# prs-eth/Marigold

Hardware: NVIDIA B200
Metric: denoise-steps/sec @768px (UNet forward + scheduler step per ensemble member) (higher is better)
Workload: dtype bf16

## Files before the change

### marigold_b200/csrc/attn_tc.cu

```cuda
#include <cstdlib>
#include "common.cuh"
#include "kernels.h"
#include "launch.h"

namespace mgb {

constexpr int attn_threads(int rt) { return 64 + 128 * rt; }
constexpr int kQBytes = 128 * 128;
constexpr int kKvBytes = 64 * 128;
constexpr int kPBytes = 128 * 128;
constexpr int kKvStages = 3;
constexpr float kRescaleThreshold = 8.0f;
constexpr int kAttnDefaultRT = 2;
struct AttnParams {
  CUtensorMap tmap_q;
  CUtensorMap tmap_kv;
  bf16* out;
  int T, C;
  float scale_log2;
  int splits;
  float* part_o;
  float* part_ml;
};

template <int N>
__device__ __forceinline__ void quarter_barrier(int q) {
  switch (q) {
    case 0: asm volatile("bar.sync 1, %0;" ::"n"(N) : "memory"); break;
    case 1: asm volatile("bar.sync 2, %0;" ::"n"(N) : "memory"); break;
    case 2: asm volatile("bar.sync 3, %0;" ::"n"(N) : "memory"); break;
    default: asm volatile("bar.sync 4, %0;" ::"n"(N) : "memory"); break;
  }
}

template <int RT>
__global__ void __launch_bounds__(attn_threads(RT), 2) flash_attn64_kernel(const __grid_constant__ AttnParams p) {
  pdl_launch_dependents();
  extern __shared__ uint8_t smem_raw[];
  uint8_t* smem = reinterpret_cast<uint8_t*>((reinterpret_cast<uintptr_t>(smem_raw) + 1023) & ~uintptr_t(1023));
  uint8_t* sQ = smem;
  uint8_t* sK = sQ + kQBytes;
  uint8_t* sV = sK + kKvStages * kKvBytes;
  uint64_t* bars = reinterpret_cast<uint64_t*>(sV + kKvStages * kKvBytes);
  uint64_t* q_full = bars;
  uint64_t* k_full = bars + 1;
  uint64_t* k_empty = bars + 4;
  uint64_t* v_full = bars + 7;
  uint64_t* v_empty = bars + 10;
  uint64_t* s_full = bars + 13;
  uint64_t* p_full = bars + 15;
  uint64_t* p_empty = bars + 17;
  uint32_t* tmem_ptr_smem = reinterpret_cast<uint32_t*>(bars + 19);
  float* s_xch = reinterpret_cast<float*>(bars + 20);

  const int warp = threadIdx.x >> 5, lane = threadIdx.x & 31;
  const int q0 = blockIdx.x * 128, head = blockIdx.y, img = blockIdx.z / p.splits, split = blockIdx.z % p.splits;
  const int nkv_all = (p.T + 63) / 64;
  const int jb0 = split * nkv_all / p.splits;
  const int nkv = (split + 1) * nkv_all / p.splits - jb0;

  if (warp == 0 && lane == 0) {
    tma_prefetch_desc(&p.tmap_q);
    tma_prefetch_desc(&p.tmap_kv);
    mbar_init(q_full, 1);
    for (int s = 0; s < kKvStages; ++s) {
      mbar_init(&k_full[s], 1); mbar_init(&k_empty[s], 1);
      mbar_init(&v_full[s], 1); mbar_init(&v_empty[s], 1);
    }
    for (int b = 0; b < 2; ++b) {
      mbar_init(&s_full[b], 1);
      mbar_init(&p_full[b], 128 * RT);
      mbar_init(&p_empty[b], 1);
    }
    fence_mbar_init();
  }
  if (warp == 1) {
    tmem_alloc(tmem_ptr_smem, 256);
    tmem_relinquish();
  }
  tc_fence_before();
  __syncthreads();
  tc_fence_after();
  const uint32_t tmem_base = *tmem_ptr_smem;
  const uint32_t tmem_o = tmem_base + 128;
  pdl_wait();

  if (warp == 0) {
    if (elect_one()) {
      const uint32_t kfull = smem_u32(k_full), kempty = smem_u32(k_empty), vfull = smem_u32(v_full),
                     vempty = smem_u32(v_empty);
      const uint32_t sK_a = smem_u32(sK), sV_a = smem_u32(sV);
      mbar_arrive_expect_tx(q_full, kQBytes);
      tma_load_3d(sQ, &p.tmap_q, q_full, head * 64, q0, img);
      const int ck = p.C + head * 64, cv = 2 * p.C + head * 64;
      uint32_t s = 0, ph = 0;
      for (int j = 0; j < nkv; ++j) {
        mbar_wait_a(kempty + s * 8, ph ^ 1);
        mbar_expect_tx_a(kfull + s * 8, kKvBytes);
        tma_load_3d_a(sK_a + s * kKvBytes, &p.tmap_kv, kfull + s * 8, ck, (jb0 + j) * 64, img);
        mbar_wait_a(vempty + s * 8, ph ^ 1);
        mbar_expect_tx_a(vfull + s * 8, kKvBytes);
        tma_load_3d_a(sV_a + s * kKvBytes, &p.tmap_kv, vfull + s * 8, cv, (jb0 + j) * 64, img);
        if (++s == kKvStages) { s = 0; ph ^= 1; }
      }
    }
  } else if (warp == 1) {
    if (elect_one()) {
      constexpr uint32_t idesc_s = umma_idesc_bf16(128, 64, false);
      constexpr uint32_t idesc_pv = umma_idesc_bf16(128, 64, true);
      constexpr uint32_t kHi = uint32_t(kDescSw128Hi >> 32), kLbo = 1u << 16;
      const uint32_t kfull = smem_u32(k_full), kempty = smem_u32(k_empty), vfull = smem_u32(v_full),
                     vempty = smem_u32(v_empty), sfull = smem_u32(s_full), pfull = smem_u32(p_full),
                     pempty = smem_u32(p_empty);
      const uint32_t dq_lo = (smem_u32(sQ) >> 4) | kLbo, dk_lo0 = (smem_u32(sK) >> 4) | kLbo,
                     dv_lo0 = (smem_u32(sV) >> 4) | kLbo;
      uint32_t ks = 0, kph = 0, vs = 0, vph = 0;
      auto issue_s = [&](int j) {
        mbar_wait_a(kfull + ks * 8, kph);
        const uint32_t dk_lo = dk_lo0 + ks * uint32_t(kKvBytes >> 4);
        const uint32_t ts = tmem_base + uint32_t(j & 1) * 64;
        umma_bf16(ts, make_u64(dq_lo, kHi), make_u64(dk_lo, kHi), idesc_s, 0u);
        umma_bf16(ts, make_u64(dq_lo + 2, kHi), make_u64(dk_lo + 2, kHi), idesc_s, 1u);
        umma_bf16(ts, make_u64(dq_lo + 4, kHi), make_u64(dk_lo + 4, kHi), idesc_s, 1u);
        umma_bf16(ts, make_u64(dq_lo + 6, kHi), make_u64(dk_lo + 6, kHi), idesc_s, 1u);
        umma_commit_a(kempty + ks * 8);
        umma_commit_a(sfull + uint32_t(j & 1) * 8);
        if (++ks == kKvStages) { ks = 0; kph ^= 1; }
      };
      mbar_wait_a(smem_u32(q_full), 0);
      issue_s(0);
      for (int j = 0; j < nkv; ++j) {
        if (j + 1 < nkv) issue_s(j + 1);
        const uint32_t b = uint32_t(j & 1);
        mbar_wait_a(pfull + b * 8, uint32_t(j >> 1) & 1u);
        mbar_wait_a(vfull + vs * 8, vph);
        tc_fence_after();
        const uint32_t tp = tmem_base + 192 + b * 32;
        const uint32_t dv_lo = dv_lo0 + vs * uint32_t(kKvBytes >> 4);
        umma_bf16_ts(tmem_o, tp, make_u64(dv_lo, kHi), idesc_pv, j > 0 ? 1u : 0u);
        umma_bf16_ts(tmem_o, tp + 8, make_u64(dv_lo + 128, kHi), idesc_pv, 1u);
        umma_bf16_ts(tmem_o, tp + 16, make_u64(dv_lo + 256, kHi), idesc_pv, 1u);
        umma_bf16_ts(tmem_o, tp + 24, make_u64(dv_lo + 384, kHi), idesc_pv, 1u);
        umma_commit_a(vempty + vs * 8);
        umma_commit_a(pempty + b * 8);
        if (++vs == kKvStages) { vs = 0; vph ^= 1; }
      }
    }
    __syncwarp();
  } else {
    constexpr int NS = 64 / RT;
    const int q = warp & 3;
    const int h = (warp - 2) >> 2;
    const int row = q * 32 + lane;
    const uint32_t lane_off = uint32_t(q * 32) << 16;
    float m_ref = 0.f, l_run = 0.f;
    for (int j = 0; j < nkv; ++j) {
      const int b = j & 1, u = j >> 1;
      mbar_wait(&s_full[b], u & 1);
      tc_fence_after();
      uint32_t r[NS];
      TmemIO<NS>::ld(tmem_base + lane_off + b * 64 + h * NS, r);
      tmem_wait_ld();
      const int kv_valid = p.T - (jb0 + j) * 64 - h * NS;
      if (kv_valid < NS) {
#pragma unroll
        for (int i = 0; i < NS; ++i)
          if (i >= kv_valid) r[i] = 0xff800000u;
      }
      float mxa = __uint_as_float(r[0]), mxb = __uint_as_float(r[1]), mxc = __uint_as_float(r[2]),
            mxd = __uint_as_float(r[3]);
#pragma unroll
      for (int i = 4; i < NS; i += 4) {
        mxa = fmaxf(mxa, __uint_as_float(r[i]));
        mxb = fmaxf(mxb, __uint_as_float(r[i + 1]));
        mxc = fmaxf(mxc, __uint_as_float(r[i + 2]));
        mxd = fmaxf(mxd, __uint_as_float(r[i + 3]));
      }
      float mx = fmaxf(fmaxf(mxa, mxb), fmaxf(mxc, mxd));
      float* xs = s_xch + ((b * 4 + q) * RT) * 32;
      xs[h * 32 + lane] = mx;
      quarter_barrier<32 * RT>(q);
#pragma unroll
      for (int k = 1; k < RT; ++k) mx = fmaxf(mx, xs[((h + k) % RT) * 32 + lane]);
      const float m_blk = mx * p.scale_log2;
      if (j == 0) {
        m_ref = m_blk;
      } else {
        const bool need = m_blk > m_ref + kRescaleThreshold;
        if (__any_sync(0xffffffffu, need)) {
          const float m_new = need ? m_blk : m_ref;
          const float alpha = ex2_approx(m_ref - m_new);
          m_ref = m_new;
          l_run *= alpha;
          mbar_wait(&p_empty[(j - 1) & 1], ((j - 1) >> 1) & 1);
          tc_fence_after();
          uint32_t o[NS];
          TmemIO<NS>::ld(tmem_o + lane_off + h * NS, o);
          tmem_wait_ld();
#pragma unroll
          for (int i = 0; i < NS; ++i) o[i] = __float_as_uint(__uint_as_float(o[i]) * alpha);
          TmemIO<NS>::st(tmem_o + lane_off + h * NS, o);
          tmem_wait_st();
        }
      }
      uint32_t pk[NS / 2];
      f2 ls01 = f2_splat(0.f), ls23 = ls01;
      const f2 sc2 = f2_splat(p.scale_log2), nm2 = f2_splat(-m_ref);
#pragma unroll
      for (int i = 0; i < NS / 4; ++i) {
        float t0, t1, t2, t3;
        f2_split(f2_fma(f2_make(__uint_as_float(r[4 * i]), __uint_as_float(r[4 * i + 1])), sc2, nm2), t0, t1);
        f2_split(f2_fma(f2_make(__uint_as_float(r[4 * i + 2]), __uint_as_float(r[4 * i + 3])), sc2, nm2), t2, t3);
        const float a0 = ex2_approx(t0), a1 = ex2_approx(t1), a2 = ex2_approx(t2), a3 = ex2_approx(t3);
        ls01 = f2_add(ls01, f2_make(a0, a1));
        ls23 = f2_add(ls23, f2_make(a2, a3));
        pk[2 * i] = pack_bf16x2(a0, a1);
        pk[2 * i + 1] = pack_bf16x2(a2, a3);
      }
      {
        float ls0, ls1, ls2, ls3;
        f2_split(ls01, ls0, ls1);
        f2_split(ls23, ls2, ls3);
        l_run += (ls0 + ls1) + (ls2 + ls3);
      }
      mbar_wait(&p_empty[b], (u & 1) ^ 1);
      TmemIO<NS / 2>::st(tmem_base + 192 + b * 32 + h * (NS / 2) + lane_off, pk);
      tmem_wait_st();
      tc_fence_before();
      mbar_arrive(&p_full[b]);
    }
    float* xl = s_xch + (((nkv & 1) * 4 + q) * RT) * 32;
    xl[h * 32 + lane] = l_run;
    quarter_barrier<32 * RT>(q);
    float l_tot = 0.f;
#pragma unroll
    for (int k = 0; k < RT; ++k) l_tot += xl[k * 32 + lane];
    mbar_wait(&p_empty[(nkv - 1) & 1], ((nkv - 1) >> 1) & 1);
    tc_fence_after();
    const int qrow = q0 + row;
    uint32_t o0[NS];
    TmemIO<NS>::ld(tmem_o + lane_off + h * NS, o0);
    tmem_wait_ld();
    if (qrow < p.T) {
      if (p.splits == 1) {
        const float inv = 1.f / l_tot;
        uint4* dst = reinterpret_cast<uint4*>(p.out + ((size_t)img * p.T + qrow) * p.C + head * 64 + h * NS);
#pragma unroll
        for (int i = 0; i < NS / 8; ++i)
          dst[i] = make_uint4(pack_bf16x2(__uint_as_float(o0[8 * i]) * inv, __uint_as_float(o0[8 * i + 1]) * inv),
                              pack_bf16x2(__uint_as_float(o0[8 * i + 2]) * inv, __uint_as_float(o0[8 * i + 3]) * inv),
                              pack_bf16x2(__uint_as_float(o0[8 * i + 4]) * inv, __uint_as_float(o0[8 * i + 5]) * inv),
                              pack_bf16x2(__uint_as_float(o0[8 * i + 6]) * inv, __uint_as_float(o0[8 * i + 7]) * inv));
      } else {
        const size_t prow = ((size_t(split) * gridDim.z / p.splits + img) * gridDim.y + head) * p.T + qrow;
        uint4* dst = reinterpret_cast<uint4*>(p.part_o + prow * 64 + h * NS);
#pragma unroll
        for (int i = 0; i < NS / 4; ++i) dst[i] = make_uint4(o0[4 * i], o0[4 * i + 1], o0[4 * i + 2], o0[4 * i + 3]);
        if (h == 0) *reinterpret_cast<float2*>(p.part_ml + prow * 2) = make_float2(m_ref, l_tot);
      }
    }
    tc_fence_before();
  }
  __syncthreads();
  if (warp == 1) {
    tc_fence_after();
    tmem_dealloc(tmem_base, 256);
  }
}

__global__ void __launch_bounds__(256) attn_combine_kernel(const float* __restrict__ part_o, const float* __restrict__ part_ml,
                                                           bf16* __restrict__ out, int splits, int NB, int heads, int T, int C) {
  pdl_launch_dependents();
  pdl_wait();
  const size_t rows = size_t(NB) * heads * T;
  const size_t gid = size_t(blockIdx.x) * blockDim.x + threadIdx.x;
  const size_t r = gid >> 3;
  const int c8 = int(gid & 7) * 8;
  if (r >= rows) return;
  float m = -INFINITY;
  for (int s = 0; s < splits; ++s) m = fmaxf(m, __ldg(part_ml + (size_t(s) * rows + r) * 2));
  float acc[8] = {0.f, 0.f, 0.f, 0.f, 0.f, 0.f, 0.f, 0.f}, l = 0.f;
  for (int s = 0; s < splits; ++s) {
    const float2 ml = __ldg(reinterpret_cast<const float2*>(part_ml + (size_t(s) * rows + r) * 2));
    const float w = ex2_approx(ml.x - m);
    l = fmaf(ml.y, w, l);
    const float4* po = reinterpret_cast<const float4*>(part_o + (size_t(s) * rows + r) * 64 + c8);
    const float4 a = __ldg(po), b = __ldg(po + 1);
    acc[0] = fmaf(a.x, w, acc[0]); acc[1] = fmaf(a.y, w, acc[1]); acc[2] = fmaf(a.z, w, acc[2]); acc[3] = fmaf(a.w, w, acc[3]);
    acc[4] = fmaf(b.x, w, acc[4]); acc[5] = fmaf(b.y, w, acc[5]); acc[6] = fmaf(b.z, w, acc[6]); acc[7] = fmaf(b.w, w, acc[7]);
  }
  const float inv = 1.f / l;
  const size_t t = r % T, ih = r / T;
  const size_t img = ih / heads, head = ih % heads;
  uint4* dst = reinterpret_cast<uint4*>(out + (img * T + t) * C + head * 64 + c8);
  *dst = make_uint4(pack_bf16x2(acc[0] * inv, acc[1] * inv), pack_bf16x2(acc[2] * inv, acc[3] * inv),
                    pack_bf16x2(acc[4] * inv, acc[5] * inv), pack_bf16x2(acc[6] * inv, acc[7] * inv));
}

int flash_attn64_splits(int NB, int T, int C) {
  const int units = ((T + 127) / 128) * (C / 64) * NB, nkv = (T + 63) / 64, slots = 148 * 2;
  int best = 1;
  double best_t = 1e30;
  for (int s = 1; s <= 8; ++s) {
    if (s > 1 && nkv / s < 6) break;
    const double rounds = double((units * s + slots - 1) / slots);
    const double t = rounds * (double(nkv) / s + 15.0) + (s > 1 ? 8.0 : 0.0);
    if (t < best_t - 1e-9) { best_t = t; best = s; }
  }
  return best;
}
size_t flash_attn64_ws_bytes(int NB, int T, int C) {
  const int s = flash_attn64_splits(NB, T, C);
  if (s == 1) return 0;
  return size_t(s) * NB * (C / 64) * T * (64 + 2) * sizeof(float);
}

int launch_flash_attn64(const bf16* qkv, bf16* out, int NB, int T, int C, float scale, float* ws, size_t ws_bytes,
                        cudaStream_t stream) {
  if (C % 64 != 0 || T <= 0) {
    set_error("flash_attn64: C %% 64 != 0 or bad T");
    return MGB_ERR_INVALID;
  }
  AttnParams p;
  const uint64_t dims[3] = {uint64_t(3 * C), uint64_t(T), uint64_t(NB)};
  const uint64_t strides[2] = {uint64_t(3 * C) * 2, uint64_t(T) * 3 * C * 2};
  const uint32_t box_q[3] = {64, 128, 1}, box_kv[3] = {64, 64, 1};
  int rc = make_tmap_3d(&p.tmap_q, qkv, dims, strides, box_q);
  if (rc) return rc;
  rc = make_tmap_3d(&p.tmap_kv, qkv, dims, strides, box_kv);
  if (rc) return rc;
  p.out = out; p.T = T; p.C = C;
  p.scale_log2 = scale * 1.4426950408889634f;
  p.splits = 1; p.part_o = nullptr; p.part_ml = nullptr;
  {
    const int sp = flash_attn64_splits(NB, T, C);
    if (sp > 1 && ws != nullptr && ws_bytes >= flash_attn64_ws_bytes(NB, T, C)) {
      p.splits = sp;
      p.part_o = ws;
      p.part_ml = ws + size_t(sp) * NB * (C / 64) * T * 64;
    }
  }
  static const size_t dbg_pad = getenv("MGB_ATTN_SMEM_PAD") ? size_t(atoi(getenv("MGB_ATTN_SMEM_PAD"))) : 0;
  const size_t smem = 1024 + kQBytes + 2 * kKvStages * kKvBytes + 256 + 4096 + dbg_pad;
  static const int rt = getenv("MGB_ATTN_RT") ? atoi(getenv("MGB_ATTN_RT")) : kAttnDefaultRT;
  void (*kern)(AttnParams) = rt == 4 ? flash_attn64_kernel<4> : flash_attn64_kernel<2>;
  static bool attr_set = false;
  if (!attr_set) {
    cudaError_t e = cudaFuncSetAttribute(kern, cudaFuncAttributeMaxDynamicSharedMemorySize, int(smem));
    if (e != cudaSuccess) { set_error("flash_attn64 attr: %s", cudaGetErrorString(e)); return MGB_ERR_CUDA; }
    attr_set = true;
  }
  dim3 grid((T + 127) / 128, C / 64, NB * p.splits);
  cudaError_t e = launch_k(kern, grid, attn_threads(rt == 4 ? 4 : 2), smem, stream, p);
  if (e == cudaSuccess) e = cudaGetLastError();
  if (e != cudaSuccess) { set_error("flash_attn64 launch: %s", cudaGetErrorString(e)); return MGB_ERR_CUDA; }
  if (p.splits > 1) {
    const size_t threads = size_t(NB) * (C / 64) * T * 8;
    e = launch_k(attn_combine_kernel, dim3(unsigned((threads + 255) / 256)), 256, 0, stream, (const float*)p.part_o,
                 (const float*)p.part_ml, out, p.splits, NB, C / 64, T, C);
    if (e == cudaSuccess) e = cudaGetLastError();
    if (e != cudaSuccess) { set_error("attn_combine launch: %s", cudaGetErrorString(e)); return MGB_ERR_CUDA; }
  }
  return MGB_OK;
}

}
```

Measured before the change: 210.0.

## Restructure Blackwell flash attention into dual Q-tile ping-pong with 128-wide KV blocks

Rewrites the tcgen05 attention kernel so each CTA owns two 128-row Q tiles, each processed by its own 4-warp softmax group with one thread per row, against 128-wide KV blocks. The MMA warp interleaves the S and PV matmuls of the two tiles, so tensor-core work for one tile overlaps the other tile's softmax. It also offloads part of the exponentials to an FMA polynomial, drops the cross-warp max exchange, and retunes the split-KV heuristic. In exchange it uses all 512 TMEM columns, more shared memory and one CTA per SM, and the polynomial exp slightly changes numerics.

```diff
diff --git a/marigold_b200/csrc/attn_tc.cu b/marigold_b200/csrc/attn_tc.cu
--- a/marigold_b200/csrc/attn_tc.cu
+++ b/marigold_b200/csrc/attn_tc.cu
@@ -1,88 +1,103 @@
-#include <cstdlib>
 #include "common.cuh"
 #include "kernels.h"
 #include "launch.h"
 
 namespace mgb {
 
-constexpr int attn_threads(int rt) { return 64 + 128 * rt; }
-constexpr int kQBytes = 128 * 128;
-constexpr int kKvBytes = 64 * 128;
-constexpr int kPBytes = 128 * 128;
+constexpr int kAttnThreads = 320;
+constexpr int kTileBytes = 128 * 128;
 constexpr int kKvStages = 3;
 constexpr float kRescaleThreshold = 8.0f;
-constexpr int kAttnDefaultRT = 2;
+constexpr size_t kAttnSmemBytes = 1024 + 2 * kTileBytes + 2 * kKvStages * kTileBytes + 256;
+constexpr int kAttnPolyPairs = 4;
+
 struct AttnParams {
-  CUtensorMap tmap_q;
-  CUtensorMap tmap_kv;
+  CUtensorMap tmap;
   bf16* out;
-  int T, C;
+  int T, C, NB;
   float scale_log2;
   int splits;
   float* part_o;
   float* part_ml;
 };
 
-template <int N>
-__device__ __forceinline__ void quarter_barrier(int q) {
-  switch (q) {
-    case 0: asm volatile("bar.sync 1, %0;" ::"n"(N) : "memory"); break;
-    case 1: asm volatile("bar.sync 2, %0;" ::"n"(N) : "memory"); break;
-    case 2: asm volatile("bar.sync 3, %0;" ::"n"(N) : "memory"); break;
-    default: asm volatile("bar.sync 4, %0;" ::"n"(N) : "memory"); break;
-  }
-}
-
-template <int RT>
-__global__ void __launch_bounds__(attn_threads(RT), 2) flash_attn64_kernel(const __grid_constant__ AttnParams p) {
+constexpr float kExp2C1 = 0.6951163411140442f;
+constexpr float kExp2C2 = 0.22764700651168823f;
+constexpr float kExp2C3 = 0.07706519961357117f;
+__device__ __forceinline__ f2 f2_add_rm(f2 a, f2 b) {
+  f2 r;
+  asm("add.rm.f32x2 %0, %1, %2;" : "=l"(r) : "l"(a), "l"(b));
+  return r;
+}
+__device__ __forceinline__ void exp2_poly_f2(float x0, float x1, float& y0, float& y1) {
+  const f2 x = f2_make(fmaxf(x0, -127.f), fmaxf(x1, -127.f));
+  const f2 t = f2_add_rm(x, f2_splat(12582912.f));
+  const f2 f = f2_sub(x, f2_sub(t, f2_splat(12582912.f)));
+  f2 q = f2_fma(f2_splat(kExp2C3), f, f2_splat(kExp2C2));
+  q = f2_fma(q, f, f2_splat(kExp2C1));
+  q = f2_fma(q, f, f2_splat(1.f));
+  float q0, q1, t0, t1;
+  f2_split(q, q0, q1);
+  f2_split(t, t0, t1);
+  y0 = __uint_as_float(__float_as_uint(q0) + (__float_as_uint(t0) << 23));
+  y1 = __uint_as_float(__float_as_uint(q1) + (__float_as_uint(t1) << 23));
+}
+
+__device__ __forceinline__ uint32_t addr_at_use(uint32_t base, uint32_t off) {
+  uint32_t r;
+  asm volatile("add.u32 %0, %1, %2;" : "=r"(r) : "r"(base), "r"(off));
+  return r;
+}
+
+__global__ void __launch_bounds__(kAttnThreads, 1) flash_attn64_kernel(const __grid_constant__ AttnParams p) {
   pdl_launch_dependents();
   extern __shared__ uint8_t smem_raw[];
   uint8_t* smem = reinterpret_cast<uint8_t*>((reinterpret_cast<uintptr_t>(smem_raw) + 1023) & ~uintptr_t(1023));
   uint8_t* sQ = smem;
-  uint8_t* sK = sQ + kQBytes;
-  uint8_t* sV = sK + kKvStages * kKvBytes;
-  uint64_t* bars = reinterpret_cast<uint64_t*>(sV + kKvStages * kKvBytes);
+  uint8_t* sK = sQ + 2 * kTileBytes;
+  uint8_t* sV = sK + kKvStages * kTileBytes;
+  uint64_t* bars = reinterpret_cast<uint64_t*>(sV + kKvStages * kTileBytes);
   uint64_t* q_full = bars;
   uint64_t* k_full = bars + 1;
   uint64_t* k_empty = bars + 4;
   uint64_t* v_full = bars + 7;
   uint64_t* v_empty = bars + 10;
   uint64_t* s_full = bars + 13;
-  uint64_t* p_full = bars + 15;
-  uint64_t* p_empty = bars + 17;
-  uint32_t* tmem_ptr_smem = reinterpret_cast<uint32_t*>(bars + 19);
-  float* s_xch = reinterpret_cast<float*>(bars + 20);
+  uint64_t* s_drained = bars + 15;
+  uint64_t* p_full = bars + 17;
+  uint64_t* pv_done = bars + 19;
+  uint32_t* tmem_ptr_smem = reinterpret_cast<uint32_t*>(bars + 21);
 
   const int warp = threadIdx.x >> 5, lane = threadIdx.x & 31;
-  const int q0 = blockIdx.x * 128, head = blockIdx.y, img = blockIdx.z / p.splits, split = blockIdx.z % p.splits;
-  const int nkv_all = (p.T + 63) / 64;
+  const int q0 = blockIdx.x * 256, head = blockIdx.y, img = blockIdx.z / p.splits, split = blockIdx.z % p.splits;
+  const bool has_b = q0 + 128 < p.T;
+  const int nkv_all = (p.T + 127) / 128;
   const int jb0 = split * nkv_all / p.splits;
   const int nkv = (split + 1) * nkv_all / p.splits - jb0;
 
   if (warp == 0 && lane == 0) {
-    tma_prefetch_desc(&p.tmap_q);
-    tma_prefetch_desc(&p.tmap_kv);
+    tma_prefetch_desc(&p.tmap);
     mbar_init(q_full, 1);
     for (int s = 0; s < kKvStages; ++s) {
       mbar_init(&k_full[s], 1); mbar_init(&k_empty[s], 1);
       mbar_init(&v_full[s], 1); mbar_init(&v_empty[s], 1);
     }
-    for (int b = 0; b < 2; ++b) {
-      mbar_init(&s_full[b], 1);
-      mbar_init(&p_full[b], 128 * RT);
-      mbar_init(&p_empty[b], 1);
+    for (int t = 0; t < 2; ++t) {
+      mbar_init(&s_full[t], 1);
+      mbar_init(&s_drained[t], 128);
+      mbar_init(&p_full[t], 128);
+      mbar_init(&pv_done[t], 1);
     }
     fence_mbar_init();
   }
   if (warp == 1) {
-    tmem_alloc(tmem_ptr_smem, 256);
+    tmem_alloc(tmem_ptr_smem, 512);
     tmem_relinquish();
   }
   tc_fence_before();
   __syncthreads();
   tc_fence_after();
   const uint32_t tmem_base = *tmem_ptr_smem;
-  const uint32_t tmem_o = tmem_base + 128;
   pdl_wait();
 
   if (warp == 0) {
@@ -90,173 +105,195 @@
       const uint32_t kfull = smem_u32(k_full), kempty = smem_u32(k_empty), vfull = smem_u32(v_full),
                      vempty = smem_u32(v_empty);
       const uint32_t sK_a = smem_u32(sK), sV_a = smem_u32(sV);
-      mbar_arrive_expect_tx(q_full, kQBytes);
-      tma_load_3d(sQ, &p.tmap_q, q_full, head * 64, q0, img);
+      mbar_arrive_expect_tx(q_full, has_b ? 2 * kTileBytes : kTileBytes);
+      tma_load_3d(sQ, &p.tmap, q_full, head * 64, q0, img);
+      if (has_b) tma_load_3d(sQ + kTileBytes, &p.tmap, q_full, head * 64, q0 + 128, img);
       const int ck = p.C + head * 64, cv = 2 * p.C + head * 64;
       uint32_t s = 0, ph = 0;
       for (int j = 0; j < nkv; ++j) {
         mbar_wait_a(kempty + s * 8, ph ^ 1);
-        mbar_expect_tx_a(kfull + s * 8, kKvBytes);
-        tma_load_3d_a(sK_a + s * kKvBytes, &p.tmap_kv, kfull + s * 8, ck, (jb0 + j) * 64, img);
+        mbar_expect_tx_a(kfull + s * 8, kTileBytes);
+        tma_load_3d_a(sK_a + s * kTileBytes, &p.tmap, kfull + s * 8, ck, (jb0 + j) * 128, img);
         mbar_wait_a(vempty + s * 8, ph ^ 1);
-        mbar_expect_tx_a(vfull + s * 8, kKvBytes);
-        tma_load_3d_a(sV_a + s * kKvBytes, &p.tmap_kv, vfull + s * 8, cv, (jb0 + j) * 64, img);
+        mbar_expect_tx_a(vfull + s * 8, kTileBytes);
+        tma_load_3d_a(sV_a + s * kTileBytes, &p.tmap, vfull + s * 8, cv, (jb0 + j) * 128, img);
         if (++s == kKvStages) { s = 0; ph ^= 1; }
       }
     }
   } else if (warp == 1) {
     if (elect_one()) {
-      constexpr uint32_t idesc_s = umma_idesc_bf16(128, 64, false);
+      constexpr uint32_t idesc_s = umma_idesc_bf16(128, 128, false);
       constexpr uint32_t idesc_pv = umma_idesc_bf16(128, 64, true);
       constexpr uint32_t kHi = uint32_t(kDescSw128Hi >> 32), kLbo = 1u << 16;
       const uint32_t kfull = smem_u32(k_full), kempty = smem_u32(k_empty), vfull = smem_u32(v_full),
-                     vempty = smem_u32(v_empty), sfull = smem_u32(s_full), pfull = smem_u32(p_full),
-                     pempty = smem_u32(p_empty);
-      const uint32_t dq_lo = (smem_u32(sQ) >> 4) | kLbo, dk_lo0 = (smem_u32(sK) >> 4) | kLbo,
+                     vempty = smem_u32(v_empty), sfull = smem_u32(s_full), sdrained = smem_u32(s_drained),
+                     pfull = smem_u32(p_full), pvdone = smem_u32(pv_done);
+      const uint32_t dq_lo0 = (smem_u32(sQ) >> 4) | kLbo, dk_lo0 = (smem_u32(sK) >> 4) | kLbo,
                      dv_lo0 = (smem_u32(sV) >> 4) | kLbo;
+      const int ntiles = has_b ? 2 : 1;
+      auto issue_s = [&](int t, uint32_t ks) {
+        const uint32_t dq_lo = dq_lo0 + uint32_t(t) * uint32_t(kTileBytes >> 4);
+        const uint32_t dk_lo = dk_lo0 + ks * uint32_t(kTileBytes >> 4);
+        const uint32_t ts = tmem_base + uint32_t(t) * 128;
+#pragma unroll
+        for (int k = 0; k < 4; ++k)
+          umma_bf16(ts, make_u64(dq_lo + 2 * k, kHi), make_u64(dk_lo + 2 * k, kHi), idesc_s, k > 0 ? 1u : 0u);
+        umma_commit_a(sfull + uint32_t(t) * 8);
+      };
+      auto issue_pv = [&](int t, uint32_t vs, bool acc) {
+        const uint32_t tp = tmem_base + 256 + uint32_t(t) * 64, to = tmem_base + 384 + uint32_t(t) * 64;
+        const uint32_t dv_lo = dv_lo0 + vs * uint32_t(kTileBytes >> 4);
+#pragma unroll
+        for (int k = 0; k < 8; ++k)
+          umma_bf16_ts(to, tp + 8 * k, make_u64(dv_lo + 128 * k, kHi), idesc_pv, (acc || k > 0) ? 1u : 0u);
+        umma_commit_a(pvdone + uint32_t(t) * 8);
+      };
       uint32_t ks = 0, kph = 0, vs = 0, vph = 0;
-      auto issue_s = [&](int j) {
-        mbar_wait_a(kfull + ks * 8, kph);
-        const uint32_t dk_lo = dk_lo0 + ks * uint32_t(kKvBytes >> 4);
-        const uint32_t ts = tmem_base + uint32_t(j & 1) * 64;
-        umma_bf16(ts, make_u64(dq_lo, kHi), make_u64(dk_lo, kHi), idesc_s, 0u);
-        umma_bf16(ts, make_u64(dq_lo + 2, kHi), make_u64(dk_lo + 2, kHi), idesc_s, 1u);
-        umma_bf16(ts, make_u64(dq_lo + 4, kHi), make_u64(dk_lo + 4, kHi), idesc_s, 1u);
-        umma_bf16(ts, make_u64(dq_lo + 6, kHi), make_u64(dk_lo + 6, kHi), idesc_s, 1u);
-        umma_commit_a(kempty + ks * 8);
-        umma_commit_a(sfull + uint32_t(j & 1) * 8);
-        if (++ks == kKvStages) { ks = 0; kph ^= 1; }
-      };
       mbar_wait_a(smem_u32(q_full), 0);
-      issue_s(0);
+      mbar_wait_a(kfull, 0);
+      tc_fence_after();
+      for (int t = 0; t < ntiles; ++t) issue_s(t, 0);
+      umma_commit_a(kempty);
+      ks = 1;
       for (int j = 0; j < nkv; ++j) {
-        if (j + 1 < nkv) issue_s(j + 1);
-        const uint32_t b = uint32_t(j & 1);
-        mbar_wait_a(pfull + b * 8, uint32_t(j >> 1) & 1u);
+        const uint32_t ph = uint32_t(j) & 1u;
+        const bool next = j + 1 < nkv;
+        if (next) mbar_wait_a(kfull + ks * 8, kph);
         mbar_wait_a(vfull + vs * 8, vph);
-        tc_fence_after();
-        const uint32_t tp = tmem_base + 192 + b * 32;
-        const uint32_t dv_lo = dv_lo0 + vs * uint32_t(kKvBytes >> 4);
-        umma_bf16_ts(tmem_o, tp, make_u64(dv_lo, kHi), idesc_pv, j > 0 ? 1u : 0u);
-        umma_bf16_ts(tmem_o, tp + 8, make_u64(dv_lo + 128, kHi), idesc_pv, 1u);
-        umma_bf16_ts(tmem_o, tp + 16, make_u64(dv_lo + 256, kHi), idesc_pv, 1u);
-        umma_bf16_ts(tmem_o, tp + 24, make_u64(dv_lo + 384, kHi), idesc_pv, 1u);
+        for (int t = 0; t < ntiles; ++t) {
+          if (next) {
+            mbar_wait_a(sdrained + uint32_t(t) * 8, ph);
+            tc_fence_after();
+            issue_s(t, ks);
+          }
+          mbar_wait_a(pfull + uint32_t(t) * 8, ph);
+          tc_fence_after();
+          issue_pv(t, vs, j > 0);
+        }
+        if (next) {
+          umma_commit_a(kempty + ks * 8);
+          if (++ks == kKvStages) { ks = 0; kph ^= 1; }
+        }
         umma_commit_a(vempty + vs * 8);
-        umma_commit_a(pempty + b * 8);
         if (++vs == kKvStages) { vs = 0; vph ^= 1; }
       }
     }
     __syncwarp();
-  } else {
-    constexpr int NS = 64 / RT;
-    const int q = warp & 3;
-    const int h = (warp - 2) >> 2;
-    const int row = q * 32 + lane;
-    const uint32_t lane_off = uint32_t(q * 32) << 16;
+  } else if (warp < 6 || has_b) {
+    const int t = warp >= 6 ? 1 : 0;
+    const int qw = warp & 3;
+    const int row = qw * 32 + lane;
+    const uint32_t lane_off = uint32_t(qw * 32) << 16;
+    const uint32_t tS = tmem_base + lane_off + uint32_t(t) * 128, tP = tmem_base + lane_off + 256 + uint32_t(t) * 64,
+                   tO = tmem_base + lane_off + 384 + uint32_t(t) * 64;
     float m_ref = 0.f, l_run = 0.f;
     for (int j = 0; j < nkv; ++j) {
-      const int b = j & 1, u = j >> 1;
-      mbar_wait(&s_full[b], u & 1);
+      const uint32_t ph = uint32_t(j) & 1u;
+      mbar_wait(&s_full[t], ph);
       tc_fence_after();
-      uint32_t r[NS];
-      TmemIO<NS>::ld(tmem_base + lane_off + b * 64 + h * NS, r);
+      uint32_t r[128];
+      tmem_ld32(tS, *reinterpret_cast<uint32_t(*)[32]>(r));
+      tmem_ld32(addr_at_use(tS, 32), *reinterpret_cast<uint32_t(*)[32]>(r + 32));
+      tmem_ld32(addr_at_use(tS, 64), *reinterpret_cast<uint32_t(*)[32]>(r + 64));
+      tmem_ld32(addr_at_use(tS, 96), *reinterpret_cast<uint32_t(*)[32]>(r + 96));
       tmem_wait_ld();
-      const int kv_valid = p.T - (jb0 + j) * 64 - h * NS;
-      if (kv_valid < NS) {
-#pragma unroll
-        for (int i = 0; i < NS; ++i)
+      tc_fence_before();
+      mbar_arrive(&s_drained[t]);
+      const int kv_valid = p.T - (jb0 + j) * 128;
+      if (kv_valid < 128) {
+#pragma unroll
+        for (int i = 0; i < 128; ++i)
           if (i >= kv_valid) r[i] = 0xff800000u;
       }
-      float mxa = __uint_as_float(r[0]), mxb = __uint_as_float(r[1]), mxc = __uint_as_float(r[2]),
-            mxd = __uint_as_float(r[3]);
-#pragma unroll
-      for (int i = 4; i < NS; i += 4) {
-        mxa = fmaxf(mxa, __uint_as_float(r[i]));
-        mxb = fmaxf(mxb, __uint_as_float(r[i + 1]));
-        mxc = fmaxf(mxc, __uint_as_float(r[i + 2]));
-        mxd = fmaxf(mxd, __uint_as_float(r[i + 3]));
-      }
-      float mx = fmaxf(fmaxf(mxa, mxb), fmaxf(mxc, mxd));
-      float* xs = s_xch + ((b * 4 + q) * RT) * 32;
-      xs[h * 32 + lane] = mx;
-      quarter_barrier<32 * RT>(q);
-#pragma unroll
-      for (int k = 1; k < RT; ++k) mx = fmaxf(mx, xs[((h + k) % RT) * 32 + lane]);
-      const float m_blk = mx * p.scale_log2;
+      float mx[4];
+#pragma unroll
+      for (int c = 0; c < 4; ++c) mx[c] = __uint_as_float(r[c]);
+#pragma unroll
+      for (int i = 4; i < 128; i += 4)
+#pragma unroll
+        for (int c = 0; c < 4; ++c) mx[c] = fmaxf(mx[c], __uint_as_float(r[i + c]));
+      const float m_blk = fmaxf(fmaxf(mx[0], mx[1]), fmaxf(mx[2], mx[3])) * p.scale_log2;
+      bool rescale = false;
+      float alpha = 1.f;
       if (j == 0) {
         m_ref = m_blk;
       } else {
+        mbar_wait(&pv_done[t], ph ^ 1);
+        tc_fence_after();
         const bool need = m_blk > m_ref + kRescaleThreshold;
-        if (__any_sync(0xffffffffu, need)) {
-          const float m_new = need ? m_blk : m_ref;
-          const float alpha = ex2_approx(m_ref - m_new);
-          m_ref = m_new;
+        rescale = __any_sync(0xffffffffu, need);
+        if (need) {
+          alpha = ex2_approx(m_ref - m_blk);
+          m_ref = m_blk;
           l_run *= alpha;
-          mbar_wait(&p_empty[(j - 1) & 1], ((j - 1) >> 1) & 1);
-          tc_fence_after();
-          uint32_t o[NS];
-          TmemIO<NS>::ld(tmem_o + lane_off + h * NS, o);
+        }
+      }
+      const f2 sc2 = f2_splat(p.scale_log2), nm2 = f2_splat(-m_ref);
+      f2 ls0 = f2_splat(0.f), ls1 = ls0;
+#pragma unroll
+      for (int c = 0; c < 4; ++c) {
+        uint32_t pk[16];
+#pragma unroll
+        for (int i = 0; i < 16; ++i) {
+          float t0, t1, a0, a1;
+          f2_split(f2_fma(f2_make(__uint_as_float(r[32 * c + 2 * i]), __uint_as_float(r[32 * c + 2 * i + 1])), sc2, nm2),
+                   t0, t1);
+          if (((i + 1) * kAttnPolyPairs) / 16 != (i * kAttnPolyPairs) / 16) {
+            exp2_poly_f2(t0, t1, a0, a1);
+          } else {
+            a0 = ex2_approx(t0);
+            a1 = ex2_approx(t1);
+          }
+          if (i & 1) ls1 = f2_add(ls1, f2_make(a0, a1));
+          else ls0 = f2_add(ls0, f2_make(a0, a1));
+          pk[i] = pack_bf16x2(a0, a1);
+        }
+        tmem_st16(addr_at_use(tP, c * 16), pk);
+      }
+      {
+        float s0, s1, s2, s3;
+        f2_split(ls0, s0, s1);
+        f2_split(ls1, s2, s3);
+        l_run += (s0 + s1) + (s2 + s3);
+      }
+      if (rescale) {
+#pragma unroll
+        for (int h = 0; h < 2; ++h) {
+          uint32_t o[32];
+          tmem_ld32(addr_at_use(tO, h * 32), o);
           tmem_wait_ld();
 #pragma unroll
-          for (int i = 0; i < NS; ++i) o[i] = __float_as_uint(__uint_as_float(o[i]) * alpha);
-          TmemIO<NS>::st(tmem_o + lane_off + h * NS, o);
-          tmem_wait_st();
+          for (int i = 0; i < 32; ++i) o[i] = __float_as_uint(__uint_as_float(o[i]) * alpha);
+          tmem_st32(addr_at_use(tO, h * 32), o);
         }
       }
-      uint32_t pk[NS / 2];
-      f2 ls01 = f2_splat(0.f), ls23 = ls01;
-      const f2 sc2 = f2_splat(p.scale_log2), nm2 = f2_splat(-m_ref);
-#pragma unroll
-      for (int i = 0; i < NS / 4; ++i) {
-        float t0, t1, t2, t3;
-        f2_split(f2_fma(f2_make(__uint_as_float(r[4 * i]), __uint_as_float(r[4 * i + 1])), sc2, nm2), t0, t1);
-        f2_split(f2_fma(f2_make(__uint_as_float(r[4 * i + 2]), __uint_as_float(r[4 * i + 3])), sc2, nm2), t2, t3);
-        const float a0 = ex2_approx(t0), a1 = ex2_approx(t1), a2 = ex2_approx(t2), a3 = ex2_approx(t3);
-        ls01 = f2_add(ls01, f2_make(a0, a1));
-        ls23 = f2_add(ls23, f2_make(a2, a3));
-        pk[2 * i] = pack_bf16x2(a0, a1);
-        pk[2 * i + 1] = pack_bf16x2(a2, a3);
-      }
-      {
-        float ls0, ls1, ls2, ls3;
-        f2_split(ls01, ls0, ls1);
-        f2_split(ls23, ls2, ls3);
-        l_run += (ls0 + ls1) + (ls2 + ls3);
-      }
-      mbar_wait(&p_empty[b], (u & 1) ^ 1);
-      TmemIO<NS / 2>::st(tmem_base + 192 + b * 32 + h * (NS / 2) + lane_off, pk);
       tmem_wait_st();
       tc_fence_before();
-      mbar_arrive(&p_full[b]);
-    }
-    float* xl = s_xch + (((nkv & 1) * 4 + q) * RT) * 32;
-    xl[h * 32 + lane] = l_run;
-    quarter_barrier<32 * RT>(q);
-    float l_tot = 0.f;
-#pragma unroll
-    for (int k = 0; k < RT; ++k) l_tot += xl[k * 32 + lane];
-    mbar_wait(&p_empty[(nkv - 1) & 1], ((nkv - 1) >> 1) & 1);
+      mbar_arrive(&p_full[t]);
+    }
+    mbar_wait(&pv_done[t], uint32_t(nkv - 1) & 1u);
     tc_fence_after();
-    const int qrow = q0 + row;
-    uint32_t o0[NS];
-    TmemIO<NS>::ld(tmem_o + lane_off + h * NS, o0);
+    const int qrow = q0 + t * 128 + row;
+    uint32_t o[64];
+    tmem_ld32(tO, *reinterpret_cast<uint32_t(*)[32]>(o));
+    tmem_ld32(tO + 32, *reinterpret_cast<uint32_t(*)[32]>(o + 32));
     tmem_wait_ld();
     if (qrow < p.T) {
       if (p.splits == 1) {
-        const float inv = 1.f / l_tot;
-        uint4* dst = reinterpret_cast<uint4*>(p.out + ((size_t)img * p.T + qrow) * p.C + head * 64 + h * NS);
-#pragma unroll
-        for (int i = 0; i < NS / 8; ++i)
-          dst[i] = make_uint4(pack_bf16x2(__uint_as_float(o0[8 * i]) * inv, __uint_as_float(o0[8 * i + 1]) * inv),
-                              pack_bf16x2(__uint_as_float(o0[8 * i + 2]) * inv, __uint_as_float(o0[8 * i + 3]) * inv),
-                              pack_bf16x2(__uint_as_float(o0[8 * i + 4]) * inv, __uint_as_float(o0[8 * i + 5]) * inv),
-                              pack_bf16x2(__uint_as_float(o0[8 * i + 6]) * inv, __uint_as_float(o0[8 * i + 7]) * inv));
+        const float inv = 1.f / l_run;
+        uint4* dst = reinterpret_cast<uint4*>(p.out + ((size_t)img * p.T + qrow) * p.C + head * 64);
+#pragma unroll
+        for (int i = 0; i < 8; ++i)
+          dst[i] = make_uint4(pack_bf16x2(__uint_as_float(o[8 * i]) * inv, __uint_as_float(o[8 * i + 1]) * inv),
+                              pack_bf16x2(__uint_as_float(o[8 * i + 2]) * inv, __uint_as_float(o[8 * i + 3]) * inv),
+                              pack_bf16x2(__uint_as_float(o[8 * i + 4]) * inv, __uint_as_float(o[8 * i + 5]) * inv),
+                              pack_bf16x2(__uint_as_float(o[8 * i + 6]) * inv, __uint_as_float(o[8 * i + 7]) * inv));
       } else {
-        const size_t prow = ((size_t(split) * gridDim.z / p.splits + img) * gridDim.y + head) * p.T + qrow;
-        uint4* dst = reinterpret_cast<uint4*>(p.part_o + prow * 64 + h * NS);
-#pragma unroll
-        for (int i = 0; i < NS / 4; ++i) dst[i] = make_uint4(o0[4 * i], o0[4 * i + 1], o0[4 * i + 2], o0[4 * i + 3]);
-        if (h == 0) *reinterpret_cast<float2*>(p.part_ml + prow * 2) = make_float2(m_ref, l_tot);
+        const size_t prow = ((size_t(split) * p.NB + img) * gridDim.y + head) * p.T + qrow;
+        uint4* dst = reinterpret_cast<uint4*>(p.part_o + prow * 64);
+#pragma unroll
+        for (int i = 0; i < 16; ++i) dst[i] = make_uint4(o[4 * i], o[4 * i + 1], o[4 * i + 2], o[4 * i + 3]);
+        *reinterpret_cast<float2*>(p.part_ml + prow * 2) = make_float2(m_ref, l_run);
       }
     }
     tc_fence_before();
@@ -264,7 +301,7 @@
   __syncthreads();
   if (warp == 1) {
     tc_fence_after();
-    tmem_dealloc(tmem_base, 256);
+    tmem_dealloc(tmem_base, 512);
   }
 }
 
@@ -297,14 +334,16 @@
                     pack_bf16x2(acc[4] * inv, acc[5] * inv), pack_bf16x2(acc[6] * inv, acc[7] * inv));
 }
 
+constexpr double kAttnCtaFixedBlocks = 4.0;
+constexpr double kAttnCombineBlocks = 11.0;
 int flash_attn64_splits(int NB, int T, int C) {
-  const int units = ((T + 127) / 128) * (C / 64) * NB, nkv = (T + 63) / 64, slots = 148 * 2;
+  const int units = ((T + 255) / 256) * (C / 64) * NB, nkv = (T + 127) / 128, slots = 148;
   int best = 1;
   double best_t = 1e30;
   for (int s = 1; s <= 8; ++s) {
-    if (s > 1 && nkv / s < 6) break;
+    if (s > 1 && nkv / s < 3) break;
     const double rounds = double((units * s + slots - 1) / slots);
-    const double t = rounds * (double(nkv) / s + 15.0) + (s > 1 ? 8.0 : 0.0);
+    const double t = rounds * (double(nkv) / s + kAttnCtaFixedBlocks) + (s > 1 ? kAttnCombineBlocks : 0.0);
     if (t < best_t - 1e-9) { best_t = t; best = s; }
   }
   return best;
@@ -324,12 +363,10 @@
   AttnParams p;
   const uint64_t dims[3] = {uint64_t(3 * C), uint64_t(T), uint64_t(NB)};
   const uint64_t strides[2] = {uint64_t(3 * C) * 2, uint64_t(T) * 3 * C * 2};
-  const uint32_t box_q[3] = {64, 128, 1}, box_kv[3] = {64, 64, 1};
-  int rc = make_tmap_3d(&p.tmap_q, qkv, dims, strides, box_q);
+  const uint32_t box[3] = {64, 128, 1};
+  int rc = make_tmap_3d(&p.tmap, qkv, dims, strides, box);
   if (rc) return rc;
-  rc = make_tmap_3d(&p.tmap_kv, qkv, dims, strides, box_kv);
-  if (rc) return rc;
-  p.out = out; p.T = T; p.C = C;
+  p.out = out; p.T = T; p.C = C; p.NB = NB;
   p.scale_log2 = scale * 1.4426950408889634f;
   p.splits = 1; p.part_o = nullptr; p.part_ml = nullptr;
   {
@@ -340,18 +377,15 @@
       p.part_ml = ws + size_t(sp) * NB * (C / 64) * T * 64;
     }
   }
-  static const size_t dbg_pad = getenv("MGB_ATTN_SMEM_PAD") ? size_t(atoi(getenv("MGB_ATTN_SMEM_PAD"))) : 0;
-  const size_t smem = 1024 + kQBytes + 2 * kKvStages * kKvBytes + 256 + 4096 + dbg_pad;
-  static const int rt = getenv("MGB_ATTN_RT") ? atoi(getenv("MGB_ATTN_RT")) : kAttnDefaultRT;
-  void (*kern)(AttnParams) = rt == 4 ? flash_attn64_kernel<4> : flash_attn64_kernel<2>;
   static bool attr_set = false;
   if (!attr_set) {
-    cudaError_t e = cudaFuncSetAttribute(kern, cudaFuncAttributeMaxDynamicSharedMemorySize, int(smem));
+    cudaError_t e = cudaFuncSetAttribute(flash_attn64_kernel, cudaFuncAttributeMaxDynamicSharedMemorySize,
+                                         int(kAttnSmemBytes));
     if (e != cudaSuccess) { set_error("flash_attn64 attr: %s", cudaGetErrorString(e)); return MGB_ERR_CUDA; }
     attr_set = true;
   }
-  dim3 grid((T + 127) / 128, C / 64, NB * p.splits);
-  cudaError_t e = launch_k(kern, grid, attn_threads(rt == 4 ? 4 : 2), smem, stream, p);
+  const dim3 grid((T + 255) / 256, C / 64, NB * p.splits);
+  cudaError_t e = launch_k(flash_attn64_kernel, grid, kAttnThreads, kAttnSmemBytes, stream, p);
   if (e == cudaSuccess) e = cudaGetLastError();
   if (e != cudaSuccess) { set_error("flash_attn64 launch: %s", cudaGetErrorString(e)); return MGB_ERR_CUDA; }
   if (p.splits > 1) {
```

New measurement: 219.1 (median of 6 runs). +4.4%, better.
